# Dunni3/keypoint-diffusion

Hardware: AMD Instinct MI355X
Metric: denoising steps/sec (higher is better)
Workload: dtype f32; 1 GPU; egnn_all_atom dynamics (6 EGNN layers, hidden 256, update_kp_feat; fixed receptor encoder), batch of 64 synthetic 300-atom pockets / 25-atom ligands per GPU, T=500, seeded random-init weights, every step taken from the t=T ligand state; batch_per_gpu=64, n_rec=300, n_lig=25, parallelism=dp1

## Files before the change

### include/kpd.h

```cpp
#ifndef KPD_H
#define KPD_H

#include <stdint.h>

#ifdef __cplusplus
extern "C" {
#endif

typedef enum kpd_status {
    KPD_OK = 0,
    KPD_ERR_INVALID = -1,
    KPD_ERR_CAPACITY = -2,
    KPD_ERR_WEIGHTS = -3,
    KPD_ERR_HIP = -4,
    KPD_ERR_STATE = -5
} kpd_status;

const char *kpd_last_error(void);
int kpd_version(void);
int kpd_build_flags(void);

typedef struct kpd_batch {
    int32_t B;
    int32_t n_lig, n_kp;
// ... 22 lines not shown

kpd_status kpd_build_lig_graph(const kpd_batch *batch, float ll_cutoff, int32_t ll_k, float kl_cutoff,
                               int32_t kl_k, const kpd_lig_graph *out, void *stream);

typedef struct kpd_egnn_config {
    int32_t atom_nf, rec_nf;
    int32_t n_layers, hidden_nf;
    int32_t use_tanh, norm, update_kp_feat;
    float message_norm;
    int32_t ll_k, kl_k;
    float ll_cutoff, kl_cutoff;
    float coords_range;
} kpd_egnn_config;

typedef struct kpd_egnn kpd_egnn;

kpd_status kpd_egnn_create(const kpd_egnn_config *cfg, kpd_egnn **out);
void kpd_egnn_destroy(kpd_egnn *m);
kpd_status kpd_egnn_load_weight(kpd_egnn *m, const char *name, const float *w_dev,
                                const int64_t *shape, int32_t ndim, void *stream);
kpd_status kpd_egnn_commit(kpd_egnn *m);
kpd_status kpd_egnn_reserve(kpd_egnn *m, int32_t max_B, int32_t max_n_lig, int32_t max_n_kp,
                            int32_t max_n_kk, int32_t max_lig_per_graph, int32_t max_kp_per_graph);
kpd_status kpd_egnn_forward(kpd_egnn *m, const kpd_batch *batch, const float *t_dev,
                            float *eps_h_dev, float *eps_x_dev, void *stream);
kpd_status kpd_egnn_debug_state(kpd_egnn *m, const char *what, float *out_dev, int64_t n_floats,
                                void *stream);
kpd_status kpd_egnn_profile(kpd_egnn *m, int32_t enable);
kpd_status kpd_egnn_profile_read(kpd_egnn *m, double *total_ms, int32_t *launches);
kpd_status kpd_egnn_last_counts(kpd_egnn *m, int32_t out[8], void *stream);

typedef struct kpd_egnn_trainer kpd_egnn_trainer;
kpd_status kpd_egnn_trainer_create(const kpd_egnn_config *cfg, kpd_egnn_trainer **out);
void kpd_egnn_trainer_destroy(kpd_egnn_trainer *t);
kpd_status kpd_egnn_trainer_bind(kpd_egnn_trainer *t, const char *name, const float *weight_dev, float *grad_dev,
                                 const int64_t *shape, int32_t ndim);
kpd_status kpd_egnn_trainer_reserve(kpd_egnn_trainer *t, int32_t max_B, int32_t max_n_lig, int32_t max_n_kp,
                                    int32_t max_n_kk, int32_t max_lig_per_graph, int32_t max_kp_per_graph);
kpd_status kpd_egnn_trainer_forward(kpd_egnn_trainer *t, const kpd_batch *batch, const float *t_dev, float *eps_h_dev,
                                    float *eps_x_dev, void *stream);
kpd_status kpd_egnn_trainer_backward(kpd_egnn_trainer *t, const float *d_eps_h, const float *d_eps_x, float *d_lig_h,
                                     float *d_lig_x, float *d_kp_h, float *d_kp_x, void *stream);
kpd_status kpd_egnn_trainer_profile(kpd_egnn_trainer *t, int32_t enable);
kpd_status kpd_egnn_trainer_profile_read(kpd_egnn_trainer *t, double total_ms[2], int32_t launches[2], double edges[2]);

typedef struct kpd_gvp_config {
// ... 206 lines not shown
```

### keypoint-diffusion_amd/csrc/egnn.hip

```cpp
#include <string.h>

#include <map>
#include <set>
#include <string>
#include <vector>

#include "egnn_kernels.h"
#include "egnn_wide.h"
#include "mfma_core.h"

using namespace kpd;

namespace {

struct LayerW {
    float *wp_e[4], *wx_e[4], *b_e[4], *wr_e[4], *watt[4];
    float *wp_c[4], *wx_c[4], *b_c[4], *wr_c[4], *w3[4];
    void *wh_e[4], *wh_c[4];
    void *chh_p[2][NSLOT];
    void *wh_a[2], *wh_b[2], *wh_2[2];
    float *wp_p[2][NSLOT], *wx_p[2][NSLOT], *b_p[2][NSLOT];
    float *ch_p[2][NSLOT], *wcol_p[2][NSLOT];
    float *wp_a[2], *wx_a[2], *wp_b[2], *wx_b[2], *b0[2], *wp_2[2], *wx_2[2], *b2[2], *ln_w[2], *ln_b[2];
};

const int kSrcNt[4] = {NT_LIG, NT_KP, NT_LIG, NT_KP};
const int kDstNt[4] = {NT_LIG, NT_LIG, NT_KP, NT_KP};
const int kSrcSlot[4] = {0, 0, 6, 4};
const int kDstSlot[4] = {2, 4, 2, 6};
const char *kEtName[4] = {"ll", "kl", "lk", "kk"};
const char *kNtName[2] = {"lig", "kp"};

std::vector<std::string> split(const std::string &s, char c) {
    std::vector<std::string> out;
    size_t p = 0;
    while (true) {
        size_t q = s.find(c, p);
        out.push_back(s.substr(p, q == std::string::npos ? q : q - p));
        if (q == std::string::npos) break;
        p = q + 1;
    }
    return out;
}

int et_index(const std::string &s) {
    for (int i = 0; i < 4; ++i)
        if (s == kEtName[i]) return i;
    return -1;
}
int nt_index(const std::string &s) {
    for (int i = 0; i < 2; ++i)
        if (s == kNtName[i]) return i;
    return -1;
}

}

struct kpd_egnn {
    kpd_egnn_config cfg;
    int n_et;
    int n_upd;
    bool rec_identity;
    Arena warena, ws;
    std::vector<LayerW> L;
    float *le_W0, *le_b0, *le_W1t, *le_b1;
    float *re_W0, *re_b0, *re_W1t, *re_b1;
    float *de_W0, *de_b0, *de_W1, *de_b1;
    std::set<std::string> expected, loaded;
    bool committed = false;
    int debug_layers = -1;
    bool f16_ok = true;
    float *widen_buf = nullptr;
    int *widen_map = nullptr;
    size_t widen_floats = 0, widen_ints = 0;
    int gemm_mode = 0;
    int prune_last = 1;
    bool prof_on = false;
    std::vector<hipEvent_t> prof_ev;
    size_t prof_used = 0;

    int cap_B = 0, cap_lig = 0, cap_kp = 0, cap_kk = 0, cap_ll = 0, cap_kl = 0, cap_maxlig = 0, cap_maxkp = 0;
    int tile_cap = 0, tiles_et_cap[4] = {0, 0, 0, 0};
    float *h[2], *x[2], *P[2];
    float *hn_main[4], *hn_cont[4], *xn_main[4], *xn_cont[4];
    int *bidx[2];
    float *z[2];
    int *meta, *ll_deg, *ll_off, *kl_off, *kl_pg;
    kpd_lig_graph lg;
    EgnnWide *wide = nullptr;
};

static kpd_status build_weight_arena(kpd_egnn *m) {
    const kpd_egnn_config &c = m->cfg;
    m->warena.poison_at = 2;
    m->L.assign(c.n_layers, LayerW());
    return carve(m->warena, ARENA_TAIL, [&](Carve &A) {
        for (int i = 0; i < c.n_layers; ++i) {
            LayerW &w = m->L[i];
            const std::string pre = "egnn.conv_layers." + std::to_string(i) + ".";
            for (int et = 0; et < m->n_et; ++et) {
                A(w.wp_e[et], WP_FLOATS); A(w.wx_e[et], HS); A(w.b_e[et], HS); A(w.wr_e[et], HS); A(w.watt[et], HS);
                A(w.wp_c[et], WP_FLOATS); A(w.wx_c[et], HS); A(w.b_c[et], HS); A(w.wr_c[et], HS); A(w.w3[et], HS);
                A.as<unsigned short>(w.wh_e[et], WH_HALVES); A.as<unsigned short>(w.wh_c[et], WH_HALVES);
                for (int var = 0; var < 2; ++var) {
                    const int ss = kSrcSlot[et] + var, ds = kDstSlot[et] + var;
                    A(w.wp_p[kSrcNt[et]][ss], WP_FLOATS); A(w.wx_p[kSrcNt[et]][ss], HS);
                    A(w.wp_p[kDstNt[et]][ds], WP_FLOATS); A(w.wx_p[kDstNt[et]][ds], HS); A(w.b_p[kDstNt[et]][ds], HS);
                    A(w.ch_p[kSrcNt[et]][ss], 16 * 4096); A(w.wcol_p[kSrcNt[et]][ss], HS);
                    A(w.ch_p[kDstNt[et]][ds], 16 * 4096); A(w.wcol_p[kDstNt[et]][ds], HS);
                    A.as<unsigned short>(w.chh_p[kSrcNt[et]][ss], CHH_HALVES);
                    A.as<unsigned short>(w.chh_p[kDstNt[et]][ds], CHH_HALVES);
// ... 292 lines not shown
                    }
                } else {
                    KPD_TRY(expect_shape(name, shape, ndim, {HW}));
                    KPD_TRY(copy_pad(w, HW, L.b_p[dnt][ds], HS, st));
                    KPD_TRY(scale_inplace(L.b_p[dnt][ds], HS, SILU_C, st));
                }
            } else if (tk[5] == "2") {
                if (is_w) {
                    KPD_TRY(expect_shape(name, shape, ndim, {HW, HW}));
                    KPD_TRY(pack_gemm_weight(w, HW, HW, 0, HW, var ? L.wp_c[et] : L.wp_e[et], var ? L.wx_c[et] : L.wx_e[et], st));
                } else {
                    KPD_TRY(expect_shape(name, shape, ndim, {HW}));
                    KPD_TRY(copy_pad(w, HW, var ? L.b_c[et] : L.b_e[et], HS, st));
                }
            } else {
                KPD_TRY(expect_shape(name, shape, ndim, {1, HW}));
                KPD_TRY(copy_pad(w, HW, L.w3[et], HS, st));
                KPD_TRY(scale_inplace(L.w3[et], HS, 1.0f / SILU_C, st));
            }
        }
    }
    m->loaded.insert(nm);
    m->committed = false;
    return KPD_OK;
}

extern "C" kpd_status kpd_egnn_commit(kpd_egnn *m) {
    KPD_REQUIRE(m, KPD_ERR_INVALID, "null handle");
    if (m->wide) return wide_commit(m->wide);
    for (const std::string &n : m->expected)
        if (!m->loaded.count(n)) {
            set_error("weight '%s' was never loaded (%zu of %zu loaded)", n.c_str(), m->loaded.size(), m->expected.size());
            return KPD_ERR_WEIGHTS;
        }
    F16PackScope f16_scope;
    for (LayerW &L : m->L)
        for (int et = 0; et < m->n_et; ++et) {
            KPD_TRY(patch_bias_row(L.wp_e[et], L.wx_e[et], L.b_e[et], SILU_C, BIAS_K, nullptr));
            KPD_TRY(patch_bias_row(L.wp_c[et], L.wx_c[et], L.b_c[et], SILU_C, BIAS_K, nullptr));
            KPD_TRY(pack_f16_split(L.wp_e[et], L.wh_e[et], nullptr));
            KPD_TRY(pack_f16_split(L.wp_c[et], L.wh_c[et], nullptr));
            KPD_TRY(f16_range_check_array(L.wx_e[et], KP, nullptr));
            KPD_TRY(f16_range_check_array(L.wx_c[et], KP, nullptr));
        }
    for (LayerW &L : m->L)
        for (int nt = 0; nt < 2; ++nt)
            for (int s = 0; s < NSLOT; ++s)
                if (L.ch_p[nt][s]) KPD_TRY(pack_proj_f16_split(L.ch_p[nt][s], L.chh_p[nt][s], nullptr));
    for (LayerW &L : m->L)
        for (int nt = 0; nt < m->n_upd; ++nt) {
            KPD_TRY(pack_f16_split(L.wp_a[nt], L.wh_a[nt], nullptr));
            KPD_TRY(pack_f16_split(L.wp_b[nt], L.wh_b[nt], nullptr));
// ... 10 lines not shown
                                       int32_t max_lig_pg, int32_t max_kp_pg) {
    KPD_REQUIRE(m, KPD_ERR_INVALID, "null handle");
    KPD_REQUIRE(max_B >= 1 && max_n_lig >= 1 && max_n_kp >= 1 && max_n_kk >= 0 && max_lig_pg >= 1 && max_kp_pg >= 1,
                KPD_ERR_INVALID, "reserve: non-positive size");
    if (m->wide) return wide_reserve(m->wide, max_B, max_n_lig, max_n_kp, max_n_kk, max_lig_pg, max_kp_pg);
    if (max_B <= m->cap_B && max_n_lig <= m->cap_lig && max_n_kp <= m->cap_kp && max_n_kk <= m->cap_kk &&
        max_lig_pg <= m->cap_maxlig && max_kp_pg <= m->cap_maxkp)
        return KPD_OK;
    max_B = std::max(max_B, m->cap_B); max_n_lig = std::max(max_n_lig, m->cap_lig); max_n_kp = std::max(max_n_kp, m->cap_kp);
    max_n_kk = std::max(max_n_kk, m->cap_kk); max_lig_pg = std::max(max_lig_pg, m->cap_maxlig); max_kp_pg = std::max(max_kp_pg, m->cap_maxkp);
    kpd_lig_graph &g = m->lg;
    KPD_TRY(lig_graph_caps(m->cfg.ll_k, m->cfg.kl_k, max_n_lig, max_n_kp, max_lig_pg, g));
    KPD_REQUIRE(((long)std::max(max_n_lig, max_n_kp) + TM) * NSLOT * HS * 4 < (1l << 32), KPD_ERR_CAPACITY,
                "batch of %d / %d nodes exceeds the 4 GB addressable per node type by the edge kernel's 32-bit row offsets (split the batch)",
                max_n_lig, max_n_kp);
    const int cap_ll = g.cap_ll, cap_kl = g.cap_kl;
    const int E_cap[4] = {cap_ll, cap_kl, cap_kl, std::max(max_n_kk, 1)};
    int tiles[4], tile_cap = 0;
    for (int et = 0; et < 4; ++et) {
        tiles[et] = cdiv(E_cap[et], 32) + 1;
        tile_cap += tiles[et];
    }
    const int n[2] = {max_n_lig, max_n_kp};
    KPD_TRY(carve(m->ws, ARENA_TAIL, [&](Carve &W) {
        for (int nt = 0; nt < 2; ++nt) {
            W(m->h[nt], (size_t)(n[nt] + TM) * HS);
            W(m->x[nt], (size_t)n[nt] * 3);
            W.rows(m->P[nt], (size_t)(n[nt] + TM) * NSLOT, HS, HW);
            W(m->bidx[nt], n[nt]);
            W(m->z[nt], max_B);
        }
        for (int et = 0; et < 4; ++et) {
            W.rows(m->hn_main[et], n[kDstNt[et]], HS, HW);
            W.rows(m->hn_cont[et], tiles[et], HS, HW);
            W(m->xn_main[et], (size_t)n[kDstNt[et]] * 4);
            W(m->xn_cont[et], (size_t)tiles[et] * 4);
        }
        carve_lig_graph(W, m->meta, m->ll_deg, m->ll_off, m->kl_off, m->kl_pg, g, max_B, max_n_lig, max_n_kp);
    }));
    for (int et = 0; et < 4; ++et) m->tiles_et_cap[et] = tiles[et];
    m->cap_B = max_B; m->cap_lig = max_n_lig; m->cap_kp = max_n_kp; m->cap_kk = max_n_kk;
    m->cap_ll = cap_ll; m->cap_kl = cap_kl; m->cap_maxlig = max_lig_pg; m->cap_maxkp = max_kp_pg;
    m->tile_cap = tile_cap;
    return KPD_OK;
}

extern "C" kpd_status kpd_egnn_forward(kpd_egnn *m, const kpd_batch *bt, const float *t_dev, float *eps_h, float *eps_x,
                                       void *stream) {
    KPD_REQUIRE(m && bt && t_dev && eps_h && eps_x, KPD_ERR_INVALID, "null argument");
    KPD_REQUIRE(m->wide || m->committed, KPD_ERR_STATE, "kpd_egnn_forward before kpd_egnn_commit");
    KPD_REQUIRE(bt->B >= 1 && bt->n_lig >= 1 && bt->n_kp >= 1, KPD_ERR_INVALID, "empty batch (B=%d n_lig=%d n_kp=%d)", bt->B, bt->n_lig, bt->n_kp);
    KPD_REQUIRE(!m->cfg.update_kp_feat || bt->n_kk == 0 || (bt->kk_src && bt->kk_dst), KPD_ERR_INVALID, "kk edges missing");
    KPD_REQUIRE(bt->kk_rowptr, KPD_ERR_INVALID, "kk_rowptr missing");
    if (m->wide) return wide_forward(m->wide, bt, t_dev, eps_h, eps_x, static_cast<hipStream_t>(stream));
    KPD_REQUIRE(bt->B <= m->cap_B && bt->n_lig <= m->cap_lig && bt->n_kp <= m->cap_kp && bt->n_kk <= m->cap_kk &&
                    bt->max_lig <= m->cap_maxlig && bt->max_kp <= m->cap_maxkp,
                KPD_ERR_CAPACITY, "batch (B=%d lig=%d kp=%d kk=%d maxlig=%d maxkp=%d) exceeds reserved workspace (%d %d %d %d %d %d)",
                bt->B, bt->n_lig, bt->n_kp, bt->n_kk, bt->max_lig, bt->max_kp, m->cap_B, m->cap_lig, m->cap_kp, m->cap_kk,
                m->cap_maxlig, m->cap_maxkp);
    hipStream_t st = static_cast<hipStream_t>(stream);
    const kpd_egnn_config &c = m->cfg;

    KPD_HIP(hipMemcpyAsync(m->x[NT_LIG], bt->lig_x, (size_t)bt->n_lig * 12, hipMemcpyDeviceToDevice, st));
    KPD_HIP(hipMemcpyAsync(m->x[NT_KP], bt->kp_x, (size_t)bt->n_kp * 12, hipMemcpyDeviceToDevice, st));
    KPD_TRY(launch_node_graph_index(bt->lig_ptr, bt->B, bt->n_lig, m->bidx[NT_LIG], st));
    KPD_TRY(launch_node_graph_index(bt->kp_ptr, bt->B, bt->n_kp, m->bidx[NT_KP], st));
    KPD_TRY(launch_lig_graph(bt, c.ll_cutoff, c.ll_k, c.kl_cutoff, c.kl_k, &m->lg, m->ll_deg, m->ll_off, m->kl_off, m->kl_pg, st));
    const int tr = TM;
    const int active = c.update_kp_feat ? 0xF : 0x3;
    const bool prune = c.update_kp_feat && m->prune_last;
    const int active_last = prune ? 0x3 : active;
    KPD_TRY(launch_egnn_meta(m->lg.counts, bt->n_kk, active, active_last, bt->lig_ptr, bt->kp_ptr, m->lg.ll_per_graph,
                             bt->kk_rowptr, bt->B, m->kl_off, c.message_norm, c.update_kp_feat, m->meta, m->z[NT_LIG],
                             m->z[NT_KP], st, tr));
    KPD_TRY(launch_embed(bt->lig_h, bt->n_lig, c.atom_nf, m->le_W0, m->le_b0, 64, m->le_W1t, m->le_b1, t_dev,
                         m->bidx[NT_LIG], m->h[NT_LIG], 0, st));
    KPD_TRY(launch_embed(bt->kp_h, bt->n_kp, c.rec_nf, m->re_W0, m->re_b0, 2 * c.rec_nf, m->re_W1t, m->re_b1, t_dev,
                         m->bidx[NT_KP], m->h[NT_KP], m->rec_identity ? 1 : 0, st));

    const int e_kl_cap = bt->n_kp * (c.kl_k > 0 ? c.kl_k : std::min(bt->max_lig, 100));
    const int E_cap[4] = {std::max<int>((long)bt->n_lig * std::min(bt->max_lig - 1, c.ll_k > 0 ? c.ll_k : 200), 1), e_kl_cap, e_kl_cap,
                          bt->n_kk};
    int tile_cap = 0, tile_cap_last = 0;
    for (int et = 0; et < m->n_et; ++et) {
        tile_cap += cdiv(E_cap[et], tr);
        if ((active_last >> et) & 1) tile_cap_last += cdiv(E_cap[et], tr);
    }

    const int n[2] = {bt->n_lig, bt->n_kp};
    const int *esrc[4] = {m->lg.ll_src, m->lg.kl_src, m->lg.lk_src, bt->kk_src};
    const int *edst[4] = {m->lg.ll_dst, m->lg.kl_dst, m->lg.lk_dst, bt->kk_dst};
    const int *rowptr[4] = {m->lg.ll_rowptr, m->lg.kl_rowptr, m->lg.lk_rowptr, bt->kk_rowptr};
    const int n_layers = m->debug_layers >= 0 ? std::min(m->debug_layers, c.n_layers) : c.n_layers;

    auto slot_mask = [&](int etmask, int nt) {
        int mk = 0;
        for (int et = 0; et < 4; ++et)
            if ((etmask >> et) & 1) {
                if (kSrcNt[et] == nt) mk |= 3 << kSrcSlot[et];
                if (kDstNt[et] == nt) mk |= 3 << kDstSlot[et];
            }
        return mk;
    };
    auto layer_etmask = [&](int li) { return li == n_layers - 1 ? active_last : active; };
    for (int li = 0; li < n_layers; ++li) {
        const LayerW &L = m->L[li];
        {
            {
                ProjPair pp;
                memset(&pp, 0, sizeof(pp));
                for (int nt = 0; nt < 2; ++nt) {
                    ProjArgs &pa = pp.nt[nt];
                    pa.h = m->h[nt]; pa.n = n[nt]; pa.P = m->P[nt];
                    int k = 0;
                    const int mk = slot_mask(layer_etmask(li), nt);
                    for (int s = 0; s < NSLOT; ++s)
                        if (L.wp_p[nt][s] && ((mk >> s) & 1)) {
                            pa.wp[k] = L.wp_p[nt][s]; pa.wx[k] = L.wx_p[nt][s]; pa.bias[k] = L.b_p[nt][s]; pa.slot[k] = s;
                            pa.chain[k] = L.ch_p[nt][s]; pa.wcol[k] = L.wcol_p[nt][s]; pa.chain_h[k] = L.chh_p[nt][s];
                            ++k;
                        }
                    pp.n_slots[nt] = k;
                }
                pp.tiles0 = cdiv(n[0], TM);
                pp.gemm_mode = m->gemm_mode;
                KPD_TRY(launch_proj_chain(pp, st));
            }
        }
        EdgeArgs ea;
        memset(&ea, 0, sizeof(ea));
        const bool last = li == n_layers - 1;
        ea.meta = last ? m->meta + 16 : m->meta;
        ea.x[0] = m->x[0]; ea.x[1] = m->x[1]; ea.P[0] = m->P[0]; ea.P[1] = m->P[1];
        ea.use_tanh = c.use_tanh; ea.coords_range = c.coords_range;
        ea.tile_rows = tr;
        ea.gemm_mode = tr == TM ? m->gemm_mode : 0;
        for (int et = 0; et < 4; ++et) {
            ea.src[et] = esrc[et]; ea.dst[et] = edst[et];
// ... 152 lines not shown
```

### keypoint-diffusion_amd/csrc/egnn_chain.hip

```cpp
#include <algorithm>
#include <cstdlib>

#include "chain_core.h"
#include "egnn_kernels.h"

namespace kpd {

namespace {

constexpr int ENT = 16;
constexpr int ECH4 = ENT * 64;

__device__ __forceinline__ float reduce_q(float v) {
    v += __shfl_xor(v, 16);
    v += __shfl_xor(v, 32);
    return v;
}

}

struct ProjWs {
    ProjPair p;
    int blocks0;
    int bpc[2];
// ... 240 lines not shown
    int blocks[2];
    for (q.tpb = std::max(1, cdiv(units, target));; ++q.tpb) {
        for (int nt = 0; nt < 2; ++nt) {
            q.bpc[nt] = std::max(1, cdiv(tl[nt], q.tpb));
            blocks[nt] = tl[nt] ? 2 * p.n_slots[nt] * q.bpc[nt] : 0;
        }
        if (blocks[0] + blocks[1] <= target || q.tpb >= std::max(tl[0], tl[1])) break;
    }
    q.blocks0 = blocks[0];
    if (p.gemm_mode == 1) {
        for (int nt = 0; nt < 2; ++nt)
            for (int s = 0; s < p.n_slots[nt]; ++s)
                KPD_REQUIRE(p.nt[nt].chain_h[s], KPD_ERR_STATE, "projection slot %d has no f16 planes (f16x2 mode)", s);
        KPD_TRY(ensure_dynamic_lds(reinterpret_cast<const void *>(k_proj_ws_h), WS_LDS_BYTES));
        hipLaunchKernelGGL(k_proj_ws_h, dim3(blocks[0] + blocks[1]), dim3(512), WS_LDS_BYTES, st, q);
        KPD_LAUNCH_CHECK();
        return KPD_OK;
    }
    hipLaunchKernelGGL(k_proj_ws, dim3(blocks[0] + blocks[1]), dim3(512), WS_LDS_BYTES, st, q);
    KPD_LAUNCH_CHECK();
    return KPD_OK;
}

}
```

### keypoint-diffusion_amd/csrc/egnn_kernels.h

```cpp
#pragma once
#include "engine.h"

namespace kpd {

constexpr int NSLOT = 8;
constexpr int ATT_BIAS_AT = 260;
constexpr int BIAS_K = 260;
constexpr int ET_LL = 0, ET_KL = 1, ET_LK = 2, ET_KK = 3;
constexpr int NT_LIG = 0, NT_KP = 1;

constexpr int EDGE_LDS_BYTES = TM * SA * 4 + (TM * 2 + TM + 3 * TM + TM + 3 * TM + 4 * HS + 8 + TM) * 4;
constexpr int EDGE_H_LDS_BYTES = 64 * 280 * 2 * 2 + (TM * 2 + TM + 3 * TM + TM + 3 * TM + 2 * HS + 8) * 4 + 2 * 2 * 272 * 2;

struct ProjArgs {
    const float *h;
    int n;
    float *P;
    const float *wp[NSLOT];
    const float *wx[NSLOT];
    const float *bias[NSLOT];
    int slot[NSLOT];
    const float *chain[NSLOT];
    const float *wcol[NSLOT];
    const void *chain_h[NSLOT];
// ... 129 lines not shown
kpd_status launch_egnn_edge_train(const EdgeTrainArgs &a, int tile_cap, hipStream_t st);
struct EdgePiecesSumArgs {
    const float *hn_main[4], *hn_cont[4], *xn_main[4], *xn_cont[4];
    const int *rowptr[4];
    int live[4], dst_nt[4];
    const float *zinv[2];
    int n[2];
    float *hn[2], *xn[2];
};
kpd_status launch_edge_pieces_sum(const EdgePiecesSumArgs &a, hipStream_t st);
kpd_status launch_edge_train_pack(const EdgePackTab &t, hipStream_t st);
kpd_status launch_egnn_edge_bwd(const EdgeBwdArgs &a, int tile_cap, hipStream_t st);
struct EdgePiecesBatch {
    struct One {
        const float *m1, *c1, *m2, *c2;
        const int *rowptr;
        int n;
        float *o1, *o2;
    } e[8];
    int ldo;
};
kpd_status launch_edge_pieces_set(const EdgePiecesBatch &b, int count, hipStream_t st);
kpd_status launch_proj_chain(const ProjPair &p, hipStream_t st);
kpd_status launch_node_layer(const NodeLayerPair &p, hipStream_t st);

}
```

### keypoint-diffusion_amd/hip.py

```python
import ctypes as C
import os
from typing import Dict, Optional

import torch

_HERE = os.path.dirname(os.path.abspath(__file__))
LIB_PATH = os.environ.get('KPD_LIB') or os.path.join(_HERE, 'csrc', 'libkpd_hip.so')
_lib = None

c_int_p = C.POINTER(C.c_int32)
c_float_p = C.POINTER(C.c_float)


class KpdBatch(C.Structure):
    _fields_ = [('B', C.c_int32), ('n_lig', C.c_int32), ('n_kp', C.c_int32), ('max_lig', C.c_int32),
                ('max_kp', C.c_int32), ('lig_ptr', C.c_void_p), ('kp_ptr', C.c_void_p), ('lig_x', C.c_void_p),
                ('lig_h', C.c_void_p), ('kp_x', C.c_void_p), ('kp_h', C.c_void_p), ('kp_v', C.c_void_p),
                ('n_kk', C.c_int32), ('kk_src', C.c_void_p), ('kk_dst', C.c_void_p), ('kk_rowptr', C.c_void_p)]


class KpdLigGraph(C.Structure):
    _fields_ = [('cap_ll', C.c_int32), ('cap_kl', C.c_int32),
                ('ll_src', C.c_void_p), ('ll_dst', C.c_void_p), ('ll_rowptr', C.c_void_p),
                ('kl_src', C.c_void_p), ('kl_dst', C.c_void_p), ('kl_rowptr', C.c_void_p),
# ... 54 lines not shown
    pass


def lib():
    global _lib
    if _lib is not None:
        return _lib
    if not os.path.exists(LIB_PATH):
        raise KpdError(f'{LIB_PATH} not found: the HIP extension must be built first '
                       f'(python -c "import __graft_entry__ as g; g.build()"). There is no CPU fallback.')
    L = C.CDLL(LIB_PATH)
    L.kpd_last_error.restype = C.c_char_p
    L.kpd_version.restype = C.c_int
    L.kpd_build_flags.restype = C.c_int
    for name in EXPORTS:
        getattr(L, name)
    L.kpd_egnn_create.argtypes = [C.POINTER(KpdEgnnConfig), C.POINTER(C.c_void_p)]
    L.kpd_egnn_destroy.argtypes = [C.c_void_p]
    L.kpd_egnn_destroy.restype = None
    L.kpd_egnn_load_weight.argtypes = [C.c_void_p, C.c_char_p, C.c_void_p, C.POINTER(C.c_int64), C.c_int32, C.c_void_p]
    L.kpd_egnn_commit.argtypes = [C.c_void_p]
    L.kpd_egnn_reserve.argtypes = [C.c_void_p] + [C.c_int32] * 6
    L.kpd_egnn_forward.argtypes = [C.c_void_p, C.POINTER(KpdBatch), C.c_void_p, C.c_void_p, C.c_void_p, C.c_void_p]
    L.kpd_egnn_debug_state.argtypes = [C.c_void_p, C.c_char_p, C.c_void_p, C.c_int64, C.c_void_p]
    L.kpd_egnn_last_counts.argtypes = [C.c_void_p, C.POINTER(C.c_int32), C.c_void_p]
    L.kpd_egnn_profile.argtypes = [C.c_void_p, C.c_int32]
    L.kpd_egnn_profile_read.argtypes = [C.c_void_p, C.POINTER(C.c_double), C.POINTER(C.c_int32)]
    L.kpd_gvp_create.argtypes = [C.POINTER(KpdGvpConfig), C.POINTER(C.c_void_p)]
    L.kpd_gvp_destroy.argtypes = [C.c_void_p]
    L.kpd_gvp_destroy.restype = None
    L.kpd_gvp_load_weight.argtypes = [C.c_void_p, C.c_char_p, C.c_void_p, C.POINTER(C.c_int64), C.c_int32, C.c_void_p]
    L.kpd_gvp_commit.argtypes = [C.c_void_p]
    L.kpd_gvp_reserve.argtypes = [C.c_void_p] + [C.c_int32] * 6
    L.kpd_gvp_forward.argtypes = [C.c_void_p, C.POINTER(KpdBatch), C.c_void_p, C.c_void_p, C.c_void_p, C.c_void_p]
    L.kpd_gvp_debug_state.argtypes = [C.c_void_p, C.c_char_p, C.c_void_p, C.c_int64, C.c_void_p]
    L.kpd_gvp_last_counts.argtypes = [C.c_void_p, C.POINTER(C.c_int32), C.c_void_p]
    L.kpd_gvp_profile.argtypes = [C.c_void_p, C.c_int32]
    L.kpd_gvp_profile_read.argtypes = [C.c_void_p, C.POINTER(C.c_double), C.POINTER(C.c_int32)]
    L.kpd_recenc_create.argtypes = [C.POINTER(KpdRecencConfig), C.POINTER(C.c_void_p)]
    L.kpd_recenc_destroy.argtypes = [C.c_void_p]
    L.kpd_recenc_destroy.restype = None
    L.kpd_recenc_load_weight.argtypes = [C.c_void_p, C.c_char_p, C.c_void_p, C.POINTER(C.c_int64), C.c_int32, C.c_void_p]
    L.kpd_recenc_commit.argtypes = [C.c_void_p]
    L.kpd_recenc_reserve.argtypes = [C.c_void_p] + [C.c_int32] * 4
    L.kpd_recenc_forward.argtypes = [C.c_void_p, C.POINTER(KpdRecBatch), C.POINTER(KpdRecOut), C.c_void_p]
    L.kpd_recegnn_create.argtypes = [C.POINTER(KpdRecegnnConfig), C.POINTER(C.c_void_p)]
# ... 47 lines not shown
    L.kpd_recegnn_trainer_reserve.argtypes = [C.c_void_p] + [C.c_int32] * 4
    L.kpd_recegnn_trainer_forward.argtypes = [C.c_void_p, C.POINTER(KpdRecBatch), C.c_void_p, C.POINTER(KpdRecOut), C.c_void_p, C.c_void_p,
                                              C.c_void_p]
    L.kpd_recegnn_trainer_backward.argtypes = [C.c_void_p] + [C.c_void_p] * 3
    L.kpd_ot_emd_uniform.argtypes = [C.c_int32, C.c_void_p, C.c_void_p, C.c_void_p, C.c_void_p, C.c_void_p, C.c_int32]
    L.kpd_sgemm.argtypes = [C.c_int32, C.c_int32, C.c_int32, C.c_int32, C.c_int32, C.c_float, C.c_void_p, C.c_int32, C.c_void_p, C.c_int32,
                            C.c_float, C.c_void_p, C.c_int32, C.c_void_p, C.c_void_p, C.c_int64, C.c_void_p]
    L.kpd_rec_graph_scratch_bytes.argtypes = [C.c_int32, C.c_int32]
    L.kpd_rec_graph_scratch_bytes.restype = C.c_int64
    L.kpd_build_rec_graph.argtypes = [C.c_void_p, C.c_void_p, C.c_int32, C.c_int32, C.c_int32, C.c_float, C.c_int32, C.c_void_p,
                                      C.c_int32] + [C.c_void_p] * 8
    L.kpd_xyz_scratch_bytes.argtypes = [C.c_int32, C.c_int32]
    L.kpd_xyz_scratch_bytes.restype = C.c_int64
    L.kpd_xyz_emit.argtypes = [C.c_void_p, C.c_void_p, C.c_void_p, C.c_int32, C.c_int32, C.c_int32, C.c_void_p, C.c_void_p,
                               C.c_void_p, C.c_int64, C.c_void_p, C.c_void_p, C.c_void_p, C.c_void_p]
    L.kpd_dist_hinge.argtypes = [C.c_void_p, C.c_void_p, C.c_int32, C.c_void_p, C.c_void_p, C.c_int32, C.c_int32, C.c_float] + [C.c_void_p] * 5
    _lib = L
    return L


EXPORTS = [
    'kpd_last_error', 'kpd_version', 'kpd_build_flags', 'kpd_build_lig_graph',
    'kpd_egnn_create', 'kpd_egnn_destroy', 'kpd_egnn_load_weight', 'kpd_egnn_commit', 'kpd_egnn_reserve',
    'kpd_egnn_forward', 'kpd_egnn_debug_state', 'kpd_egnn_last_counts', 'kpd_egnn_profile',
    'kpd_egnn_profile_read', 'kpd_sample_update', 'kpd_step_coefficients', 'kpd_complex_noise',
    'kpd_gvp_create', 'kpd_gvp_destroy', 'kpd_gvp_load_weight', 'kpd_gvp_commit', 'kpd_gvp_reserve',
    'kpd_gvp_forward', 'kpd_gvp_debug_state', 'kpd_gvp_profile', 'kpd_gvp_profile_read', 'kpd_gvp_last_counts',
    'kpd_recenc_create', 'kpd_recenc_destroy', 'kpd_recenc_load_weight', 'kpd_recenc_commit', 'kpd_recenc_reserve',
    'kpd_recenc_forward',
    'kpd_recegnn_create', 'kpd_recegnn_destroy', 'kpd_recegnn_load_weight', 'kpd_recegnn_commit', 'kpd_recegnn_reserve',
    'kpd_recegnn_forward',
    'kpd_xyz_scratch_bytes', 'kpd_xyz_emit', 'kpd_rec_graph_scratch_bytes', 'kpd_build_rec_graph',
    'kpd_egnn_trainer_create', 'kpd_egnn_trainer_destroy', 'kpd_egnn_trainer_bind', 'kpd_egnn_trainer_reserve',
    'kpd_egnn_trainer_forward', 'kpd_egnn_trainer_backward', 'kpd_egnn_trainer_profile', 'kpd_egnn_trainer_profile_read', 'kpd_gvp_trainer_last_counts',
    'kpd_gvp_trainer_message_path', 'kpd_wgrad_batch', 'kpd_adam_step',
    'kpd_gvp_trainer_create', 'kpd_gvp_trainer_destroy', 'kpd_gvp_trainer_bind', 'kpd_gvp_trainer_reserve',
    'kpd_gvp_trainer_forward', 'kpd_gvp_trainer_backward', 'kpd_gvp_trainer_set_dropout', 'kpd_dropout_mask',
    'kpd_recenc_trainer_create', 'kpd_recenc_trainer_destroy', 'kpd_recenc_trainer_bind', 'kpd_recenc_trainer_set_dropout',
    'kpd_recenc_trainer_reserve', 'kpd_recenc_trainer_forward', 'kpd_recenc_trainer_backward',
    'kpd_recegnn_trainer_create', 'kpd_recegnn_trainer_destroy', 'kpd_recegnn_trainer_bind', 'kpd_recegnn_trainer_reserve',
    'kpd_recegnn_trainer_forward', 'kpd_recegnn_trainer_backward', 'kpd_ot_emd_uniform', 'kpd_sgemm',
    'kpd_dist_hinge',
]


def check(status: int):
    if status != 0:
# ... 83 lines not shown
            _lib.kpd_egnn_destroy(self._h)
            self._h = None

    def load_state_dict(self, sd: Dict[str, torch.Tensor]):
        L = lib()
        st = _stream()
        keep = []
        for name, t in sd.items():
            t = _dev_f32(t.detach(), name)
            keep.append(t)
            shape = (C.c_int64 * t.dim())(*t.shape)
            check(L.kpd_egnn_load_weight(self._h, name.encode(), t.data_ptr(), shape, t.dim(), st))
        torch.cuda.current_stream().synchronize()
        check(L.kpd_egnn_commit(self._h))

    def reserve(self, pb: PreparedBatch):
        key = (pb.B, pb.n_lig, pb.n_kp, pb.n_kk, pb.max_lig, pb.max_kp)
        if self._reserved is not None and all(a <= b for a, b in zip(key, self._reserved)):
            return
        torch.cuda.synchronize()
        check(lib().kpd_egnn_reserve(self._h, *key))
        self._reserved = key if self._reserved is None else tuple(max(a, b) for a, b in zip(key, self._reserved))

    def forward(self, pb: PreparedBatch, lig_x, lig_h, kp_x, kp_h, t):
        self.reserve(pb)
        lig_x, lig_h = _dev_f32(lig_x, 'lig x_0'), _dev_f32(lig_h, 'lig h_0')
        kp_x, kp_h = _dev_f32(kp_x, 'kp x_0'), _dev_f32(kp_h, 'kp h_0')
        if tuple(lig_h.shape) != (pb.n_lig, self.atom_nf) or tuple(kp_h.shape) != (pb.n_kp, self.rec_nf):
            raise KpdError(f'feature shapes lig {tuple(lig_h.shape)} / kp {tuple(kp_h.shape)} do not match the denoiser '
                           f'(expected ({pb.n_lig}, atom_nf={self.atom_nf}) / ({pb.n_kp}, rec_nf={self.rec_nf}))')
        t = _dev_f32(t, 'timestep')
        eps_h = torch.empty(pb.n_lig, self.atom_nf, device=lig_x.device)
        eps_x = torch.empty(pb.n_lig, 3, device=lig_x.device)
        bt = pb.struct(lig_x, lig_h, kp_x, kp_h)
        check(lib().kpd_egnn_forward(self._h, C.byref(bt), t.data_ptr(), eps_h.data_ptr(), eps_x.data_ptr(), _stream()))
        return eps_h, eps_x

    def debug(self, what: str, n_floats: int = 0, device=None) -> Optional[torch.Tensor]:
        out = torch.empty(max(n_floats, 1), device=device or 'cuda')
        check(lib().kpd_egnn_debug_state(self._h, what.encode(), out.data_ptr(), n_floats, _stream()))
        return out if n_floats else None

    def profile(self, enable: bool):
        check(lib().kpd_egnn_profile(self._h, int(enable)))

    def profile_read(self):
        ms, n = C.c_double(), C.c_int32()
        check(lib().kpd_egnn_profile_read(self._h, C.byref(ms), C.byref(n)))
        return ms.value, n.value

    def last_counts(self):
        arr = (C.c_int32 * 8)()
        check(lib().kpd_egnn_last_counts(self._h, arr, _stream()))
        return dict(E_ll=arr[0], E_kl=arr[1], E_lk=arr[2], E_kk=arr[3], tiles=arr[4], tiles_last=arr[5], E_last=arr[6])

    def gemm_mode(self) -> str:
# ... 642 lines not shown
```

### keypoint-diffusion_amd/ligand_diffuser.py

```python
import pickle
from math import ceil
from pathlib import Path
from typing import Dict, List, Optional, Tuple

import numpy as np
import torch
import torch.nn as nn
import torch.nn.functional as F

from . import graph as G
from . import hip
from .dynamics import LigRecDynamics
from .dist_hinge_loss import segmented_dist_hinge
from .dynamics_gvp import LigRecDynamicsGVP
from .receptor_encoder_fixed import FixedReceptorEncoder
from .receptor_encoder import ReceptorEncoder
from .receptor_encoder_gvp import ReceptorEncoderGVP
from .rec_encoder_loss import ReceptorEncoderLoss


class LigandSizeDistribution:

    def __init__(self, processed_dataset_dir: Path):
        f = Path(processed_dataset_dir) / 'train_n_node_joint_dist.pkl'
# ... 53 lines not shown
            if not (t.is_contiguous() and t.dtype == torch.float32):
                raise hip.KpdError('graph capture needs contiguous fp32 state tensors (they are updated in place)')
        saved = [t.clone() for t in state]
        T = model.n_timesteps
        self.s.fill_((T - 1) / T)
        side = torch.cuda.Stream(device=dev)
        side.wait_stream(torch.cuda.current_stream(dev))
        with torch.cuda.stream(side):
            for _ in range(2):
                model.sample_p_zs_given_zt(self.s, self.t, g, bidx, noise=noise)
        torch.cuda.current_stream(dev).wait_stream(side)
        for t, c in zip(state, saved):
            t.copy_(c)
        self.graph = torch.cuda.CUDAGraph()
        with torch.cuda.graph(self.graph):
            model.sample_p_zs_given_zt(self.s, self.t, g, bidx, noise=noise)
        self._keep = (g, noise)
        self._model = model
        self._engine = model.dynamics.engine()
        self._pin = (self._engine._reserved, model.dynamics._weights_key())
        ps = list(model.dynamics.parameters())
        self._sentinels = [ps[i] for i in sorted({0, len(ps) // 2, len(ps) - 1})] if ps else []
        self._sentinel_key = [(p.data_ptr(), p._version) for p in self._sentinels]

    def _check_pin(self):
        dyn = self._model.dynamics
        self._replays = getattr(self, '_replays', -1) + 1
        if dyn._engine is not self._engine or self._engine._reserved != self._pin[0]:
            raise hip.KpdError('stale step graph: the denoiser engine was rebuilt or its workspace re-reserved (a larger batch ran) '
                               'after capture; the captured kernels point into freed memory -- capture the step again')
        if ([(p.data_ptr(), p._version) for p in self._sentinels] != self._sentinel_key or
                (self._replays % 16 == 0 and dyn._weights_key() != self._pin[1])):
            raise hip.KpdError('stale step graph: the model weights changed after capture (the graph replays the weights packed at '
                               'capture time) -- capture the step again')

    def step(self, s: float, t: float):
        self._check_pin()
        self.s.fill_(s)
        self.t.fill_(t)
        self.graph.replay()


class KeypointDiffusion(nn.Module):

    def __init__(self, atom_nf, rec_nf, processed_dataset_dir: Optional[Path], n_timesteps: int = 1000,
                 keypoint_centered=False, architecture: str = 'egnn', rec_encoder_type: str = 'learned',
                 graph_config={}, dynamics_config={}, rec_encoder_config={}, rec_encoder_loss_config={},
                 precision=1e-4, lig_feat_norm_constant=1, rl_dist_threshold=0, use_fake_atoms=False):
        super().__init__()
        if architecture not in ('egnn', 'gvp'):
            raise ValueError(f'Unsupported architecture: {architecture}')
        if rec_encoder_type not in ('learned', 'fixed'):
            raise ValueError(f'Receptor encoder type must be either "learned" or "fixed". Got {rec_encoder_type=} instead.')
        self.n_lig_features, self.n_kp_feat, self.n_timesteps = atom_nf, rec_nf, n_timesteps
        self.lig_feat_norm_constant = lig_feat_norm_constant
        self.use_fake_atoms, self.rec_encoder_type, self.architecture = use_fake_atoms, rec_encoder_type, architecture
        self.rl_dist_threshold = rl_dist_threshold
        if use_fake_atoms:
            raise NotImplementedError('fake atoms are unused by every shipped config (max_fake_atom_frac: 0.0) and '
                                      'the reference implementation of their removal cannot run (ligand_diffuser.py:559)')
# ... 275 lines not shown
```

Baseline: 152.1 steps/s.

## Cache receptor keypoint embedding and layer-0 projections across denoising steps

Adds a keypoint cache that runs the receptor embedding and the layer-0 keypoint projection chain once, with t set to zero. The cache is keyed on the keypoint feature tensor's pointer and version and on the batch layout. Each forward then runs a small elementwise kernel that adds the timestep-dependent column (t times the weight column plus bias) onto the cached projections, instead of redoing the embedding and the layer-0 keypoint GEMMs. This removes per-step receptor-side work, which is invariant over a sampling trajectory. It adds workspace memory and invalidation logic across weight loads, commits, reserves and graph capture.

```diff
diff --git a/include/kpd.h b/include/kpd.h
--- a/include/kpd.h
+++ b/include/kpd.h
@@ -68,6 +68,7 @@
 kpd_status kpd_egnn_commit(kpd_egnn *m);
 kpd_status kpd_egnn_reserve(kpd_egnn *m, int32_t max_B, int32_t max_n_lig, int32_t max_n_kp,
                             int32_t max_n_kk, int32_t max_lig_per_graph, int32_t max_kp_per_graph);
+kpd_status kpd_egnn_kp_cache(kpd_egnn *m, const kpd_batch *batch, const int64_t *key, int32_t n_key, void *stream);
 kpd_status kpd_egnn_forward(kpd_egnn *m, const kpd_batch *batch, const float *t_dev,
                             float *eps_h_dev, float *eps_x_dev, void *stream);
 kpd_status kpd_egnn_debug_state(kpd_egnn *m, const char *what, float *out_dev, int64_t n_floats,
diff --git a/keypoint-diffusion_amd/csrc/egnn.hip b/keypoint-diffusion_amd/csrc/egnn.hip
--- a/keypoint-diffusion_amd/csrc/egnn.hip
+++ b/keypoint-diffusion_amd/csrc/egnn.hip
@@ -41,6 +41,16 @@
         p = q + 1;
     }
     return out;
+}
+
+int proj_slot_mask(int etmask, int nt) {
+    int mk = 0;
+    for (int et = 0; et < 4; ++et)
+        if ((etmask >> et) & 1) {
+            if (kSrcNt[et] == nt) mk |= 3 << kSrcSlot[et];
+            if (kDstNt[et] == nt) mk |= 3 << kDstSlot[et];
+        }
+    return mk;
 }
 
 int et_index(const std::string &s) {
@@ -87,6 +97,11 @@
     float *z[2];
     int *meta, *ll_deg, *ll_off, *kl_off, *kl_pg;
     kpd_lig_graph lg;
+    float *kp_h0, *kp_P0, *kp_coef, *kp_t0;
+    bool kp_valid = false, kp_armed = false;
+    std::vector<int64_t> kp_key;
+    const float *kp_src = nullptr;
+    int kp_n = 0;
     EgnnWide *wide = nullptr;
 };
 
@@ -425,12 +440,14 @@
     }
     m->loaded.insert(nm);
     m->committed = false;
+    m->kp_valid = m->kp_armed = false;
     return KPD_OK;
 }
 
 extern "C" kpd_status kpd_egnn_commit(kpd_egnn *m) {
     KPD_REQUIRE(m, KPD_ERR_INVALID, "null handle");
     if (m->wide) return wide_commit(m->wide);
+    m->kp_valid = m->kp_armed = false;
     for (const std::string &n : m->expected)
         if (!m->loaded.count(n)) {
             set_error("weight '%s' was never loaded (%zu of %zu loaded)", n.c_str(), m->loaded.size(), m->expected.size());
@@ -487,6 +504,7 @@
         tile_cap += tiles[et];
     }
     const int n[2] = {max_n_lig, max_n_kp};
+    m->kp_valid = m->kp_armed = false;
     KPD_TRY(carve(m->ws, ARENA_TAIL, [&](Carve &W) {
         for (int nt = 0; nt < 2; ++nt) {
             W(m->h[nt], (size_t)(n[nt] + TM) * HS);
@@ -502,6 +520,10 @@
             W(m->xn_cont[et], (size_t)tiles[et] * 4);
         }
         carve_lig_graph(W, m->meta, m->ll_deg, m->ll_off, m->kl_off, m->kl_pg, g, max_B, max_n_lig, max_n_kp);
+        W(m->kp_h0, (size_t)(max_n_kp + TM) * HS);
+        W.rows(m->kp_P0, (size_t)(max_n_kp + TM) * NSLOT, HS, HW);
+        W(m->kp_coef, (size_t)NSLOT * 2 * HS);
+        W(m->kp_t0, max_B);
     }));
     for (int et = 0; et < 4; ++et) m->tiles_et_cap[et] = tiles[et];
     m->cap_B = max_B; m->cap_lig = max_n_lig; m->cap_kp = max_n_kp; m->cap_kk = max_n_kk;
@@ -510,9 +532,64 @@
     return KPD_OK;
 }
 
+static kpd_status kp_cache_fill(kpd_egnn *m, const kpd_batch *bt, hipStream_t st) {
+    const kpd_egnn_config &c = m->cfg;
+    const LayerW &L = m->L[0];
+    KPD_HIP(hipMemsetAsync(m->kp_t0, 0, (size_t)bt->B * 4, st));
+    KPD_TRY(launch_node_graph_index(bt->kp_ptr, bt->B, bt->n_kp, m->bidx[NT_KP], st));
+    KPD_TRY(launch_embed(bt->kp_h, bt->n_kp, c.rec_nf, m->re_W0, m->re_b0, 2 * c.rec_nf, m->re_W1t, m->re_b1, m->kp_t0,
+                         m->bidx[NT_KP], m->kp_h0, m->rec_identity ? 1 : 0, st));
+    ProjPair pp;
+    memset(&pp, 0, sizeof(pp));
+    ProjArgs &pa = pp.nt[NT_KP];
+    pa.h = m->kp_h0; pa.n = bt->n_kp; pa.P = m->kp_P0;
+    const int mk = proj_slot_mask(c.update_kp_feat ? 0xF : 0x3, NT_KP);
+    int k = 0;
+    for (int s = 0; s < NSLOT; ++s)
+        if (L.wp_p[NT_KP][s] && ((mk >> s) & 1)) {
+            pa.wp[k] = L.wp_p[NT_KP][s]; pa.wx[k] = L.wx_p[NT_KP][s]; pa.bias[k] = nullptr; pa.slot[k] = s;
+            pa.chain[k] = L.ch_p[NT_KP][s]; pa.wcol[k] = L.wcol_p[NT_KP][s]; pa.chain_h[k] = L.chh_p[NT_KP][s];
+            ++k;
+            float *cw = m->kp_coef + (size_t)s * 2 * HS, *cb = cw + HS;
+            KPD_HIP(hipMemcpyAsync(cw, L.wcol_p[NT_KP][s], HID * 4, hipMemcpyDeviceToDevice, st));
+            KPD_HIP(hipMemcpyAsync(cw + HID, L.wx_p[NT_KP][s] + HID, 4, hipMemcpyDeviceToDevice, st));
+            if (L.b_p[NT_KP][s]) KPD_HIP(hipMemcpyAsync(cb, L.b_p[NT_KP][s], HW * 4, hipMemcpyDeviceToDevice, st));
+            else KPD_HIP(hipMemsetAsync(cb, 0, HW * 4, st));
+        }
+    pp.n_slots[NT_KP] = k;
+    pp.gemm_mode = 0;
+    return launch_proj_chain(pp, st);
+}
+
+extern "C" kpd_status kpd_egnn_kp_cache(kpd_egnn *m, const kpd_batch *bt, const int64_t *key, int32_t n_key, void *stream) {
+    KPD_REQUIRE(m, KPD_ERR_INVALID, "null handle");
+    m->kp_armed = false;
+    if (m->wide || !key) return KPD_OK;
+    KPD_REQUIRE(bt && n_key >= 1 && n_key <= 16, KPD_ERR_INVALID, "kp cache: null batch or %d key words (1 .. 16)", n_key);
+    KPD_REQUIRE(m->committed, KPD_ERR_STATE, "kpd_egnn_kp_cache before kpd_egnn_commit");
+    KPD_REQUIRE(bt->B >= 1 && bt->n_kp >= 1 && bt->kp_h && bt->kp_ptr, KPD_ERR_INVALID, "kp cache: empty batch");
+    KPD_REQUIRE(m->ws.base && bt->B <= m->cap_B && bt->n_kp <= m->cap_kp, KPD_ERR_CAPACITY,
+                "kp cache: batch (B=%d kp=%d) exceeds the reserved workspace (%d %d)", bt->B, bt->n_kp, m->cap_B, m->cap_kp);
+    hipStream_t st = static_cast<hipStream_t>(stream);
+    const std::vector<int64_t> k(key, key + n_key);
+    if (!(m->kp_valid && k == m->kp_key && bt->kp_h == m->kp_src && bt->n_kp == m->kp_n)) {
+        hipStreamCaptureStatus cs = hipStreamCaptureStatusNone;
+        KPD_HIP(hipStreamIsCapturing(st, &cs));
+        if (cs != hipStreamCaptureStatusNone) return KPD_OK;
+        m->kp_valid = false;
+        KPD_TRY(kp_cache_fill(m, bt, st));
+        m->kp_key = k; m->kp_src = bt->kp_h; m->kp_n = bt->n_kp;
+        m->kp_valid = true;
+    }
+    m->kp_armed = true;
+    return KPD_OK;
+}
+
 extern "C" kpd_status kpd_egnn_forward(kpd_egnn *m, const kpd_batch *bt, const float *t_dev, float *eps_h, float *eps_x,
                                        void *stream) {
     KPD_REQUIRE(m && bt && t_dev && eps_h && eps_x, KPD_ERR_INVALID, "null argument");
+    const bool armed = m->kp_armed;
+    m->kp_armed = false;
     KPD_REQUIRE(m->wide || m->committed, KPD_ERR_STATE, "kpd_egnn_forward before kpd_egnn_commit");
     KPD_REQUIRE(bt->B >= 1 && bt->n_lig >= 1 && bt->n_kp >= 1, KPD_ERR_INVALID, "empty batch (B=%d n_lig=%d n_kp=%d)", bt->B, bt->n_lig, bt->n_kp);
     KPD_REQUIRE(!m->cfg.update_kp_feat || bt->n_kk == 0 || (bt->kk_src && bt->kk_dst), KPD_ERR_INVALID, "kk edges missing");
@@ -525,6 +602,7 @@
                 m->cap_maxlig, m->cap_maxkp);
     hipStream_t st = static_cast<hipStream_t>(stream);
     const kpd_egnn_config &c = m->cfg;
+    const bool kp_cached = armed && m->kp_valid && m->gemm_mode == 0 && bt->kp_h == m->kp_src && bt->n_kp == m->kp_n;
 
     KPD_HIP(hipMemcpyAsync(m->x[NT_LIG], bt->lig_x, (size_t)bt->n_lig * 12, hipMemcpyDeviceToDevice, st));
     KPD_HIP(hipMemcpyAsync(m->x[NT_KP], bt->kp_x, (size_t)bt->n_kp * 12, hipMemcpyDeviceToDevice, st));
@@ -540,8 +618,9 @@
                              m->z[NT_KP], st, tr));
     KPD_TRY(launch_embed(bt->lig_h, bt->n_lig, c.atom_nf, m->le_W0, m->le_b0, 64, m->le_W1t, m->le_b1, t_dev,
                          m->bidx[NT_LIG], m->h[NT_LIG], 0, st));
-    KPD_TRY(launch_embed(bt->kp_h, bt->n_kp, c.rec_nf, m->re_W0, m->re_b0, 2 * c.rec_nf, m->re_W1t, m->re_b1, t_dev,
-                         m->bidx[NT_KP], m->h[NT_KP], m->rec_identity ? 1 : 0, st));
+    if (!kp_cached)
+        KPD_TRY(launch_embed(bt->kp_h, bt->n_kp, c.rec_nf, m->re_W0, m->re_b0, 2 * c.rec_nf, m->re_W1t, m->re_b1, t_dev,
+                             m->bidx[NT_KP], m->h[NT_KP], m->rec_identity ? 1 : 0, st));
 
     const int e_kl_cap = bt->n_kp * (c.kl_k > 0 ? c.kl_k : std::min(bt->max_lig, 100));
     const int E_cap[4] = {std::max<int>((long)bt->n_lig * std::min(bt->max_lig - 1, c.ll_k > 0 ? c.ll_k : 200), 1), e_kl_cap, e_kl_cap,
@@ -558,16 +637,17 @@
     const int *rowptr[4] = {m->lg.ll_rowptr, m->lg.kl_rowptr, m->lg.lk_rowptr, bt->kk_rowptr};
     const int n_layers = m->debug_layers >= 0 ? std::min(m->debug_layers, c.n_layers) : c.n_layers;
 
-    auto slot_mask = [&](int etmask, int nt) {
-        int mk = 0;
-        for (int et = 0; et < 4; ++et)
-            if ((etmask >> et) & 1) {
-                if (kSrcNt[et] == nt) mk |= 3 << kSrcSlot[et];
-                if (kDstNt[et] == nt) mk |= 3 << kDstSlot[et];
-            }
-        return mk;
-    };
     auto layer_etmask = [&](int li) { return li == n_layers - 1 ? active_last : active; };
+    if (kp_cached) {
+        KpLayer0Args ka;
+        memset(&ka, 0, sizeof(ka));
+        ka.h_cache = m->kp_h0; ka.P_cache = m->kp_P0; ka.coef = m->kp_coef; ka.t = t_dev; ka.bidx = m->bidx[NT_KP];
+        ka.h = m->h[NT_KP]; ka.P = m->P[NT_KP]; ka.n = bt->n_kp;
+        const int mk = proj_slot_mask(layer_etmask(0), NT_KP);
+        for (int s = 0; s < NSLOT; ++s)
+            if (m->L[0].wp_p[NT_KP][s] && ((mk >> s) & 1)) ka.slot_map |= (unsigned)s << (4 * ka.n_slots++);
+        KPD_TRY(launch_kp_layer0(ka, st));
+    }
     for (int li = 0; li < n_layers; ++li) {
         const LayerW &L = m->L[li];
         {
@@ -578,7 +658,7 @@
                     ProjArgs &pa = pp.nt[nt];
                     pa.h = m->h[nt]; pa.n = n[nt]; pa.P = m->P[nt];
                     int k = 0;
-                    const int mk = slot_mask(layer_etmask(li), nt);
+                    const int mk = li == 0 && nt == NT_KP && kp_cached ? 0 : proj_slot_mask(layer_etmask(li), nt);
                     for (int s = 0; s < NSLOT; ++s)
                         if (L.wp_p[nt][s] && ((mk >> s) & 1)) {
                             pa.wp[k] = L.wp_p[nt][s]; pa.wx[k] = L.wx_p[nt][s]; pa.bias[k] = L.b_p[nt][s]; pa.slot[k] = s;
diff --git a/keypoint-diffusion_amd/csrc/egnn_chain.hip b/keypoint-diffusion_amd/csrc/egnn_chain.hip
--- a/keypoint-diffusion_amd/csrc/egnn_chain.hip
+++ b/keypoint-diffusion_amd/csrc/egnn_chain.hip
@@ -286,4 +286,43 @@
     return KPD_OK;
 }
 
-}
+constexpr int KP0_Q = HS / 4;
+
+__global__ __launch_bounds__(256) void k_kp_layer0(KpLayer0Args a) {
+    const long per_row = (long)(a.n_slots + 1) * KP0_Q;
+    const long i = (long)blockIdx.x * 256 + threadIdx.x;
+    if (i >= (long)a.n * per_row) return;
+    const int row = (int)(i / per_row), rem = (int)(i - row * per_row), k = rem / KP0_Q, j = rem - k * KP0_Q;
+    const float t = a.t[a.bidx[row]];
+    if (k == a.n_slots) {
+        v4f v = *reinterpret_cast<const v4f *>(a.h_cache + (size_t)row * HS + 4 * j);
+        if (j == HID / 4) v[0] = t;
+        *reinterpret_cast<v4f *>(a.h + (size_t)row * HS + 4 * j) = v;
+        return;
+    }
+    const int s = (a.slot_map >> (4 * k)) & 15;
+    const size_t off = ((size_t)row * NSLOT + s) * HS + 4 * j;
+    v4f v = *reinterpret_cast<const v4f *>(a.P_cache + off);
+    const float *cw = a.coef + (size_t)s * 2 * HS, *cb = cw + HS;
+    if (j < HID / 4) {
+        const v4f w = *reinterpret_cast<const v4f *>(cw + 4 * j), b = *reinterpret_cast<const v4f *>(cb + 4 * j);
+#pragma unroll
+        for (int r = 0; r < 4; ++r) v[r] += fmaf(t, w[r], b[r]);
+    } else if (j == HID / 4) {
+        v[0] += fmaf(t, cw[HID], cb[HID]);
+    }
+    *reinterpret_cast<v4f *>(a.P + off) = v;
+}
+
+kpd_status launch_kp_layer0(const KpLayer0Args &a, hipStream_t st) {
+    KPD_REQUIRE(a.n_slots >= 0 && a.n_slots <= NSLOT, KPD_ERR_INVALID, "kp layer 0: %d slots", a.n_slots);
+    for (int k = 0; k < a.n_slots; ++k)
+        KPD_REQUIRE(((a.slot_map >> (4 * k)) & 15) < NSLOT, KPD_ERR_INVALID, "kp layer 0: slot map %x", a.slot_map);
+    if (a.n <= 0) return KPD_OK;
+    const long threads = (long)a.n * (a.n_slots + 1) * KP0_Q;
+    hipLaunchKernelGGL(k_kp_layer0, dim3((unsigned)((threads + 255) / 256)), dim3(256), 0, st, a);
+    KPD_LAUNCH_CHECK();
+    return KPD_OK;
+}
+
+}
diff --git a/keypoint-diffusion_amd/csrc/egnn_kernels.h b/keypoint-diffusion_amd/csrc/egnn_kernels.h
--- a/keypoint-diffusion_amd/csrc/egnn_kernels.h
+++ b/keypoint-diffusion_amd/csrc/egnn_kernels.h
@@ -175,6 +175,14 @@
 };
 kpd_status launch_edge_pieces_set(const EdgePiecesBatch &b, int count, hipStream_t st);
 kpd_status launch_proj_chain(const ProjPair &p, hipStream_t st);
+struct KpLayer0Args {
+    const float *h_cache, *P_cache, *coef, *t;
+    const int *bidx;
+    float *h, *P;
+    int n, n_slots;
+    unsigned slot_map;
+};
+kpd_status launch_kp_layer0(const KpLayer0Args &a, hipStream_t st);
 kpd_status launch_node_layer(const NodeLayerPair &p, hipStream_t st);
 
 }
diff --git a/keypoint-diffusion_amd/hip.py b/keypoint-diffusion_amd/hip.py
--- a/keypoint-diffusion_amd/hip.py
+++ b/keypoint-diffusion_amd/hip.py
@@ -100,6 +100,7 @@
     L.kpd_egnn_commit.argtypes = [C.c_void_p]
     L.kpd_egnn_reserve.argtypes = [C.c_void_p] + [C.c_int32] * 6
     L.kpd_egnn_forward.argtypes = [C.c_void_p, C.POINTER(KpdBatch), C.c_void_p, C.c_void_p, C.c_void_p, C.c_void_p]
+    L.kpd_egnn_kp_cache.argtypes = [C.c_void_p, C.POINTER(KpdBatch), C.POINTER(C.c_int64), C.c_int32, C.c_void_p]
     L.kpd_egnn_debug_state.argtypes = [C.c_void_p, C.c_char_p, C.c_void_p, C.c_int64, C.c_void_p]
     L.kpd_egnn_last_counts.argtypes = [C.c_void_p, C.POINTER(C.c_int32), C.c_void_p]
     L.kpd_egnn_profile.argtypes = [C.c_void_p, C.c_int32]
@@ -193,7 +194,7 @@
 EXPORTS = [
     'kpd_last_error', 'kpd_version', 'kpd_build_flags', 'kpd_build_lig_graph',
     'kpd_egnn_create', 'kpd_egnn_destroy', 'kpd_egnn_load_weight', 'kpd_egnn_commit', 'kpd_egnn_reserve',
-    'kpd_egnn_forward', 'kpd_egnn_debug_state', 'kpd_egnn_last_counts', 'kpd_egnn_profile',
+    'kpd_egnn_forward', 'kpd_egnn_kp_cache', 'kpd_egnn_debug_state', 'kpd_egnn_last_counts', 'kpd_egnn_profile',
     'kpd_egnn_profile_read', 'kpd_sample_update', 'kpd_step_coefficients', 'kpd_complex_noise',
     'kpd_gvp_create', 'kpd_gvp_destroy', 'kpd_gvp_load_weight', 'kpd_gvp_commit', 'kpd_gvp_reserve',
     'kpd_gvp_forward', 'kpd_gvp_debug_state', 'kpd_gvp_profile', 'kpd_gvp_profile_read', 'kpd_gvp_last_counts',
@@ -323,9 +324,25 @@
         check(lib().kpd_egnn_reserve(self._h, *key))
         self._reserved = key if self._reserved is None else tuple(max(a, b) for a, b in zip(key, self._reserved))
 
-    def forward(self, pb: PreparedBatch, lig_x, lig_h, kp_x, kp_h, t):
+    def kp_cache(self, pb: PreparedBatch, kp_h: torch.Tensor, src: Optional[torch.Tensor] = None, enable: bool = True):
+        kp_h = _dev_f32(kp_h, 'kp h_0')
+        if tuple(kp_h.shape) != (pb.n_kp, self.rec_nf):
+            raise KpdError(f'kp feature shape {tuple(kp_h.shape)} does not match the denoiser (expected ({pb.n_kp}, {self.rec_nf}))')
+        self.reserve(pb)
+        src = kp_h if src is None else src
+        key = None
+        if enable and src is kp_h and not kp_h.is_inference():
+            key = (kp_h.data_ptr(), kp_h._version, pb.n_kp, self.rec_nf, pb.B, pb.kp_ptr.data_ptr(), pb.kp_ptr._version)
+        bt = pb.struct(None, None, None, kp_h)
+        arr = None if key is None else (C.c_int64 * len(key))(*key)
+        check(lib().kpd_egnn_kp_cache(self._h, C.byref(bt), arr, len(key) if key else 0, _stream()))
+        if key is not None:
+            self._kp_keep = (kp_h, pb)
+
+    def forward(self, pb: PreparedBatch, lig_x, lig_h, kp_x, kp_h, t, kp_cache: bool = True):
         self.reserve(pb)
         lig_x, lig_h = _dev_f32(lig_x, 'lig x_0'), _dev_f32(lig_h, 'lig h_0')
+        kp_src = kp_h
         kp_x, kp_h = _dev_f32(kp_x, 'kp x_0'), _dev_f32(kp_h, 'kp h_0')
         if tuple(lig_h.shape) != (pb.n_lig, self.atom_nf) or tuple(kp_h.shape) != (pb.n_kp, self.rec_nf):
             raise KpdError(f'feature shapes lig {tuple(lig_h.shape)} / kp {tuple(kp_h.shape)} do not match the denoiser '
@@ -333,6 +350,7 @@
         t = _dev_f32(t, 'timestep')
         eps_h = torch.empty(pb.n_lig, self.atom_nf, device=lig_x.device)
         eps_x = torch.empty(pb.n_lig, 3, device=lig_x.device)
+        self.kp_cache(pb, kp_h, kp_src, enable=kp_cache)
         bt = pb.struct(lig_x, lig_h, kp_x, kp_h)
         check(lib().kpd_egnn_forward(self._h, C.byref(bt), t.data_ptr(), eps_h.data_ptr(), eps_x.data_ptr(), _stream()))
         return eps_h, eps_x
diff --git a/keypoint-diffusion_amd/ligand_diffuser.py b/keypoint-diffusion_amd/ligand_diffuser.py
--- a/keypoint-diffusion_amd/ligand_diffuser.py
+++ b/keypoint-diffusion_amd/ligand_diffuser.py
@@ -99,6 +99,8 @@
         ps = list(model.dynamics.parameters())
         self._sentinels = [ps[i] for i in sorted({0, len(ps) // 2, len(ps) - 1})] if ps else []
         self._sentinel_key = [(p.data_ptr(), p._version) for p in self._sentinels]
+        kp_h = kp['h_0']
+        self._kp = (kp_h, kp_h._version) if hasattr(self._engine, 'kp_cache') and not kp_h.is_inference() else None
 
     def _check_pin(self):
         dyn = self._model.dynamics
@@ -113,6 +115,10 @@
 
     def step(self, s: float, t: float):
         self._check_pin()
+        if self._kp is not None and self._kp[0]._version != self._kp[1]:
+            kp_h = self._kp[0]
+            self._engine.kp_cache(self._keep[0].prepared(), kp_h)
+            self._kp = (kp_h, kp_h._version)
         self.s.fill_(s)
         self.t.fill_(t)
         self.graph.replay()
```

Measured after the change: 154.3 steps/s (median of 6 runs). +1.4%, better.
